# HowToSD/cremage

Hardware: AMD Instinct MI355X
Metric: images/sec SD1.5 512x512 20-step Euler ancestral (txt2img, CFG 7.5, incl. VAE decode) (higher is better)
Workload: dtype bf16; 1 GPU; SD1.5 txt2img 512x512, batch 4 per GPU, 20-step Euler ancestral, bf16 UNet (B=8 with CFG) + fp32-class (split-bf16 x3) VAE decode, synthetic name-keyed weights, synthetic conditioning; sampler=euler_a, sampler_steps=20, parallelism=batch-sharded x1 (weights broadcast 0.00 GB once, images all-gathered per step)

## Files before the change

### cremage_amd/_lib.py

```python
import ctypes as C
import os

_HERE = os.path.dirname(os.path.abspath(__file__))
HALF_F16 = os.environ.get("CRG_HALF", "bf16").lower() in ("f16", "fp16", "float16", "half")
LIB_PATH = os.path.abspath(os.environ["CRG_LIB"]) if os.environ.get("CRG_LIB") else os.path.join(_HERE, "libcrg_hip_f16.so" if HALF_F16 else "libcrg_hip.so")

BF16, F32, F16 = 0, 1, 2
PREC_BF16, PREC_BF16X3, PREC_F16MX = 0, 1, 2
EPI_NONE, EPI_SILU, EPI_GEGLU = 0, 1, 2
BIAS_NONE, BIAS_COL, BIAS_ROW = 0, 1, 2
PACK_LINEAR, PACK_CONV, PACK_GEGLU, PACK_CONV_UP2, PACK_CONVT_UP2 = 0, 1, 2, 3, 4
K_SLOTS = 17
SLOT_NAMES = ["gemm_w1", "gemm_w4", "gemm_w5", "gemm_x3", "conv_w1", "conv_w4", "conv_w5", "conv_x3", "splitk_reduce", "attention",
              "gn_stats", "gn_apply", "layernorm", "elementwise", "conv_small", "softmax", "lngemm"]
SLOT_FAMILY = ["gemm", "gemm", "gemm", "gemm", "conv", "conv", "conv", "conv", "splitk_reduce", "attention", "groupnorm", "groupnorm",
               "layernorm", "elementwise", "conv_small", "softmax", "gemm"]

c_void_p, c_int, c_int64, c_float, c_size_t = C.c_void_p, C.c_int, C.c_int64, C.c_float, C.c_size_t


class GemmArgs(C.Structure):
    _fields_ = [
        ("a", c_void_p), ("lda", c_int64), ("a_bstride", c_int64),
        ("w", c_void_p), ("ldw", c_int64), ("w_bstride", c_int64),
# ... 243 lines not shown
                                    c_int, c_float, c_int]),
    "crg_groupnorm_pre_split": (c_int, [c_void_p, c_void_p, c_void_p, c_void_p, c_void_p, c_void_p, c_void_p, c_void_p, c_int, c_int, c_int, c_int,
                                        c_float, c_int]),
    "crg_groupnorm_pre": (c_int, [c_void_p, c_void_p, c_void_p, c_void_p, c_int, c_void_p, c_void_p, c_void_p, c_void_p, c_void_p, c_int, c_int,
                                  c_int, c_int, c_float, c_int, c_int, c_int, c_int]),
    "crg_split_bf16": (c_int, [c_void_p, c_void_p, c_void_p, c_void_p, c_void_p, c_int64]),
    "crg_split_mx": (c_int, [c_void_p, c_void_p, c_void_p, c_void_p, c_void_p, c_int64, c_int, c_int, c_int]),
    "crg_groupnorm_mx": (c_int, [c_void_p, c_void_p, c_void_p, c_void_p, c_void_p, c_void_p, c_void_p, c_void_p, c_int, c_int, c_int, c_int, c_float,
                                 c_int, c_int, c_int]),
    "crg_pack_weight_mx": (c_int, [c_void_p, c_void_p, c_void_p, c_int, c_int, c_int, c_void_p, c_void_p, c_int, c_int]),
    "crg_layernorm": (c_int, [c_void_p, c_void_p, c_void_p, c_void_p, c_void_p, c_void_p, c_int64, c_int, c_float, c_int]),
    "crg_gemm": (c_int, [c_void_p, c_void_p, C.POINTER(GemmArgs)]),
    "crg_conv2d": (c_int, [c_void_p, c_void_p, C.POINTER(ConvArgs)]),
    "crg_last_route": (c_int, [c_void_p, C.POINTER(Route)]),
    "crg_ln_gemm": (c_int, [c_void_p, c_void_p, C.POINTER(LnGemmArgs)]),
    "crg_pack_weight": (c_int, [c_void_p, c_void_p, c_void_p, c_int, c_int, c_int, c_int, c_int, c_void_p, c_void_p]),
    "crg_pack_geglu_bias": (c_int, [c_void_p, c_void_p, c_void_p, c_int, c_void_p]),
    "crg_pack_ln_weight": (c_int, [c_void_p, c_void_p, c_void_p, c_int, c_void_p, c_void_p, c_void_p, c_int, c_int, c_int, c_void_p, c_void_p, c_void_p]),
    "crg_attention": (c_int, [c_void_p, c_void_p, c_void_p, c_int64, c_void_p, c_int64, c_void_p, c_int64, c_void_p, c_int64,
                              c_int, c_int, c_int, c_int, c_int, c_float, c_int]),
    "crg_attention_v": (c_int, [c_void_p, c_void_p, c_void_p, c_int64, c_void_p, c_int64, c_void_p, c_int64, c_void_p, c_int64,
                              c_int, c_int, c_int, c_int, c_int, c_float, c_int]),
    "crg_softmax_rows": (c_int, [c_void_p, c_void_p, c_void_p, c_void_p, c_int64, c_int, c_int64, c_float, c_int]),
    "crg_conv_small": (c_int, [c_void_p, c_void_p, c_void_p, c_void_p, c_void_p, c_void_p, c_int, c_int, c_int, c_int, c_int,
                               c_int, c_int, c_int]),
    "crg_timestep_embedding": (c_int, [c_void_p, c_void_p, c_void_p, c_void_p, c_int, c_int, c_int]),
    "crg_silu": (c_int, [c_void_p, c_void_p, c_void_p, c_void_p, c_int64, c_int]),
    "crg_nchw_to_nhwc": (c_int, [c_void_p, c_void_p, c_void_p, c_void_p, c_int, c_int, c_int, c_int, c_int]),
    "crg_nhwc_to_nchw": (c_int, [c_void_p, c_void_p, c_void_p, c_void_p, c_int, c_int, c_int, c_int, c_int]),
    "crg_nchw2_to_nhwc": (c_int, [c_void_p, c_void_p, c_void_p, c_void_p, c_void_p, c_int, c_int, c_int, c_int, c_int, c_int]),
# ... 131 lines not shown
```

### cremage_amd/csrc/crg_common.h

```cpp
#pragma once
#include <hip/hip_runtime.h>
#include <stdint.h>
#include <stdarg.h>
#include <stdio.h>
#include <string>
#include <vector>

#include "../../include/crg_hip.h"

#ifdef CRG_F16_BUILD
typedef _Float16 bf16;
#define CRG_HALF_KIND 1
#define CRG_MFMA_16x16x32(a, b, c) __builtin_amdgcn_mfma_f32_16x16x32_f16(a, b, c, 0, 0, 0)
#define CRG_MFMA_32x32x16(a, b, c) __builtin_amdgcn_mfma_f32_32x32x16_f16(a, b, c, 0, 0, 0)
#else
typedef __bf16 bf16;
#define CRG_HALF_KIND 0
#define CRG_MFMA_16x16x32(a, b, c) __builtin_amdgcn_mfma_f32_16x16x32_bf16(a, b, c, 0, 0, 0)
#define CRG_MFMA_32x32x16(a, b, c) __builtin_amdgcn_mfma_f32_32x32x16_bf16(a, b, c, 0, 0, 0)
#endif
typedef bf16 bf16x2 __attribute__((ext_vector_type(2)));
typedef bf16 bf16x4 __attribute__((ext_vector_type(4)));
typedef bf16 bf16x8 __attribute__((ext_vector_type(8)));
typedef float f32x2 __attribute__((ext_vector_type(2)));
// ... 38 lines not shown
  ~crg_prof_scope();
};

#define CRG_CHECK_LAUNCH(ctx, what)                                                    \
  do {                                                                                 \
    hipError_t e_ = hipGetLastError();                                                 \
    if (e_ != hipSuccess) return crg_fail(ctx, -5, "%s: launch failed: %s", what, hipGetErrorString(e_)); \
  } while (0)

#define CRG_REQUIRE(ctx, cond, ...)                         \
  do {                                                      \
    if (!(cond)) return crg_fail(ctx, -22, __VA_ARGS__);    \
  } while (0)

static inline size_t crg_dtype_size(int dt) { return dt == CRG_F32 ? 4 : 2; }

static inline int crg_set_dyn_lds(crg_ctx* ctx, const void* kern, size_t bytes, const char* what) {
  for (const void* k : ctx->lds_attr)
    if (k == kern) return 0;
  hipError_t e = hipFuncSetAttribute(kern, hipFuncAttributeMaxDynamicSharedMemorySize, (int)bytes);
  if (e != hipSuccess) return crg_fail(ctx, -5, "%s: cannot set %zu B dynamic LDS: %s", what, bytes, hipGetErrorString(e));
  ctx->lds_attr.push_back(kern);
  return 0;
}

__device__ __forceinline__ float crg_silu_f(float x) { return x * __builtin_amdgcn_rcpf(1.0f + __expf(-x)); }
__device__ __forceinline__ float crg_erf_f(float x) {
  const float ax = __builtin_fabsf(x);
  const float t = __builtin_amdgcn_rcpf(__builtin_fmaf(0.3275911f, ax, 1.0f));
  float q = __builtin_fmaf(1.061405429f, t, -1.453152027f);
// ... 72 lines not shown
```

### cremage_amd/csrc/lngemm.hip

```cpp
#include "gemm_shared.h"
#include <stdlib.h>

namespace crg_mm {

struct LnGemmP {
  const bf16* x; long ldx;
  const float* gamma; const float* beta; float eps;
  const bf16* w; long ldw;
  const float* bias;
  const bf16* res; long ldr; unsigned res_bytes;
  bf16* y; long ldy;
  int M, N, K, epi;
  unsigned x_bytes, w_bytes, y_bytes;
  bf16* vt; int vt_n0, vt_T; long vt_ld; unsigned vt_bytes;
};

#ifdef CRG_LN_ABL_NOSTORE
constexpr bool LN_DROP8 = true;
#else
constexpr bool LN_DROP8 = false;
#endif
static __device__ __forceinline__ void ln_wait(int n) {
  switch (n) {
    case 0: wait_vmcnt<0>(); break;
    case 1: wait_vmcnt<1>(); break;
    case 2: wait_vmcnt<2>(); break;
    case 3: wait_vmcnt<3>(); break;
    case 4: wait_vmcnt<4>(); break;
    case 5: wait_vmcnt<5>(); break;
// ... 40 lines not shown
    case 46: wait_vmcnt<46>(); break;
    case 47: wait_vmcnt<47>(); break;
    default: wait_vmcnt<0>(); break;
  }
}

template <int EXTRA>
static __device__ __forceinline__ void ln_wait_nw(int nW) {
  if (nW == 2) wait_vmcnt<2 + EXTRA>();
  else if (nW == 3) wait_vmcnt<3 + EXTRA>();
  else if (nW == 4) wait_vmcnt<4 + EXTRA>();
  else if (nW == 1) wait_vmcnt<1 + EXTRA>();
  else ln_wait(nW + EXTRA);
}

template <int WNT, int KT, bool GEGLU>
__global__ __launch_bounds__(512, 2) void lngemm_kernel(LnGemmP p) {
  constexpr bool PAIR = !GEGLU;
  constexpr int WMT = 2, NW = 8, BMR = 128, WST = 4;
  constexpr int BN = 32 * WNT;
  constexpr int WS_BYTES = BN * 128;
  constexpr int WRG = BN / 8;
  constexpr int WL = (WRG + NW - 1) / NW;
  constexpr int A_KT = BMR * 128;
  constexpr int AP = KT * 16 / NW;
  static_assert((KT * 16) % NW == 0, "A pieces must divide over the waves");
  constexpr int OOB = (int)0x80000000;
  extern __shared__ __attribute__((aligned(16))) char smem[];
  char* const Ares = smem;
  char* const wring = smem + KT * A_KT;

  const int t = threadIdx.x;
  const int lane = t & 63;
  const int wave = __builtin_amdgcn_readfirstlane(t >> 6);
  const int wm = wave >> 1, wn = wave & 1;
  const int m0 = blockIdx.x * BMR;
  const int rsub = lane >> 3;
  const int clog = (lane & 7) ^ rsub;
  const int frow = lane & 15, fq = lane >> 4;
  const int nW = (WRG - wave + NW - 1) / NW;
  const int tiles_n = (p.N + BN - 1) / BN;
  const int U = tiles_n * KT;
  constexpr int NST = GEGLU ? WMT * (WNT / 2) : WMT * (WNT / 2 + (WNT & 1));
  constexpr int NSTT = WMT * (8 * (WNT / 2) + 4 * (WNT & 1));

#pragma unroll
  for (int i = 0; i < AP; ++i) {
    const int pa = wave + NW * i;
    const int kt = pa >> 4, rg = pa & 15;
    const int row = m0 + rg * 8 + rsub;
    const int vo = row < p.M ? (int)((long)row * p.ldx * 2) + clog * 16 : OOB;
    buf_dma16(p.x, p.x_bytes, Ares + kt * A_KT + rg * 1024, vo, kt * 128);
  }
  int wvo[WL];
#pragma unroll
  for (int q = 0; q < WL; ++q) {
    const int pos = (wave + NW * q) * 8 + rsub;
    const int nl = PAIR ? unpair_col<WNT>(pos) : pos;
    wvo[q] = (wave + NW * q) < WRG ? (int)((long)nl * p.ldw * 2) + clog * 16 : OOB;
  }
  auto stage_w = [&](int u) {
    const int nt = u / KT, kt = u - nt * KT;
    char* ws = wring + (u & 3) * WS_BYTES;
    const int soff = (int)((long)nt * BN * p.ldw * 2) + kt * 128;
#pragma unroll
    for (int q = 0; q < WL; ++q)
      if ((wave + NW * q) < WRG) buf_dma16(p.w, p.w_bytes, ws + (wave + NW * q) * 1024, wvo[q], soff);
  };
  stage_w(0);
  stage_w(1);
  stage_w(2);

  if (p.gamma) {
    const int c = lane & 7, r8 = lane >> 3;
    f32x4 g0[KT], g1[KT], b0[KT], b1[KT];
#pragma unroll
    for (int kt = 0; kt < KT; ++kt) {
      const int k = kt * 64 + c * 8;
      g0[kt] = *reinterpret_cast<const f32x4*>(p.gamma + k);
      g1[kt] = *reinterpret_cast<const f32x4*>(p.gamma + k + 4);
      b0[kt] = *reinterpret_cast<const f32x4*>(p.beta + k);
      b1[kt] = *reinterpret_cast<const f32x4*>(p.beta + k + 4);
    }
    ln_wait(nW * 3);
    asm volatile("" ::: "memory");
    __builtin_amdgcn_s_barrier();
    asm volatile("" ::: "memory");
    const float inv_k = 1.0f / (float)(KT * 64);
// ... 30 lines not shown
#pragma unroll
        for (int e = 0; e < 8; ++e) {
          const float ga = e < 4 ? g0[kt][e] : g1[kt][e - 4], be = e < 4 ? b0[kt][e] : b1[kt][e - 4];
          o[e] = (bf16)(((float)v[kt][e] - mean) * rstd * ga + be);
        }
        *reinterpret_cast<bf16x8*>(Ares + kt * A_KT + lds_off(row, c)) = o;
      }
    }
  }

  f32x4 acc[WNT][WMT];
#pragma unroll
  for (int i = 0; i < WNT; ++i)
#pragma unroll
    for (int j = 0; j < WMT; ++j) acc[i][j] = f32x4{0.f, 0.f, 0.f, 0.f};
  const int wb0 = (wn * (16 * WNT) + frow) * 128 + ((fq ^ (frow & 7)) << 4);
  int aoff[WMT];
#pragma unroll
  for (int j = 0; j < WMT; ++j) aoff[j] = lds_off(wm * 32 + j * 16 + frow, fq);

  bf16x8 xa[KT][2][WMT];
  bf16x8 wf0[WNT], wf1[WNT];
  auto read_frags = [&](bf16x8 (&wf)[WNT], int slot, int ks) {
    const char* wbase = wring + slot * WS_BYTES + (wb0 ^ (ks << 6));
#pragma unroll
    for (int i = 0; i < WNT; ++i) wf[i] = *reinterpret_cast<const bf16x8*>(wbase + i * 2048);
  };
  auto mma = [&](const bf16x8 (&xf)[WMT], const bf16x8 (&wf)[WNT]) {
#pragma unroll
    for (int i = 0; i < WNT; ++i)
#pragma unroll
      for (int j = 0; j < WMT; ++j) acc[i][j] = CRG_MFMA_16x16x32(wf[i], xf[j], acc[i][j]);
  };
  {
    ln_wait(nW * 2);
    asm volatile("" ::: "memory");
    __builtin_amdgcn_s_barrier();
    asm volatile("" ::: "memory");
#pragma unroll
    for (int kt = 0; kt < KT; ++kt)
#pragma unroll
      for (int ks = 0; ks < 2; ++ks)
#pragma unroll
        for (int j = 0; j < WMT; ++j) xa[kt][ks][j] = *reinterpret_cast<const bf16x8*>(Ares + kt * A_KT + (aoff[j] ^ (ks << 6)));
    read_frags(wf0, 0, 0);
  }
  for (int nt = 0; nt < tiles_n; ++nt) {
// ... 14 lines not shown
      asm volatile("" ::: "memory");
      __builtin_amdgcn_s_barrier();
      asm volatile("" ::: "memory");
      read_frags(wf1, u & 3, 1);
      __builtin_amdgcn_sched_barrier(0);
#ifndef CRG_LN_ABL_NOMMA
      mma(xa[kt][0], wf0);
#endif
      __builtin_amdgcn_sched_barrier(0);
#ifndef CRG_LN_ABL_NODMA
      stage_w(u + 3);
#endif
      read_frags(wf0, (u + 1) & 3, 0);
      __builtin_amdgcn_sched_barrier(0);
#ifndef CRG_LN_ABL_NOMMA
      mma(xa[kt][1], wf1);
#else
      asm volatile("" ::"v"(wf1[0]), "v"(wf0[0]));
#endif
    }
    {
      constexpr int OOBS = (int)0x80000000;
      const int nb = n0 + wn * (16 * WNT);
      if constexpr (GEGLU) {
#pragma unroll
        for (int u2 = 0; u2 < WNT / 2; ++u2) {
          const int pn = nb + u2 * 32 + fq * 4;
          const int jn = nb / 2 + u2 * 16 + fq * 4;
          const bool nok = pn + 20 <= p.N;
          f32x4 bv = {0.f, 0.f, 0.f, 0.f}, bg = bv;
          if (p.bias) {
            const int pc = nok ? pn : 0;
            bv = *reinterpret_cast<const f32x4*>(p.bias + pc);
            bg = *reinterpret_cast<const f32x4*>(p.bias + pc + 16);
          }
#pragma unroll
          for (int j = 0; j < WMT; ++j) {
            const int m = m0 + wm * 32 + j * 16 + frow;
            const f32x4 v = acc[2 * u2][j] + bv, g = acc[2 * u2 + 1][j] + bg;
            bf16x4 o;
#pragma unroll
            for (int e = 0; e < 4; ++e) o[e] = (bf16)(v[e] * crg_gelu_erf_f(g[e]));
            buf_store8<LN_DROP8>(p.y, p.y_bytes, (nok && m < p.M) ? (int)(((long)m * p.ldy + jn) * 2) : OOBS, o);
          }
        }
      } else if (p.vt && n0 >= p.vt_n0) {
        const int Cv = p.N - p.vt_n0;
#pragma unroll
        for (int j = 0; j < WMT; ++j) {
          const int m = m0 + wm * 32 + j * 16 + frow;
          const int bs = m / p.vt_T, tk = m - bs * p.vt_T;
          const long row0 = (long)bs * Cv - p.vt_n0;
#pragma unroll
          for (int u2 = 0; u2 < WNT / 2; ++u2) {
            const int n = nb + 32 * u2 + 8 * fq;
#pragma unroll
            for (int e = 0; e < 8; ++e) {
              const float v = e < 4 ? acc[2 * u2][j][e] : acc[2 * u2 + 1][j][e - 4];
              const float bsv = p.bias ? p.bias[n + e < p.N ? n + e : 0] : 0.f;
// ... 359 lines not shown
    CRG_CHECK_LAUNCH(ctx, "ln_gemm");
    return 0;
  }
  if (geglu) { kern = lngemm_kernel<4, 5, true>; bn = 128; }
  else if (wide) { kern = lngemm_kernel<5, 5, false>; bn = 160; }
  else { kern = lngemm_kernel<4, 5, false>; bn = 128; }
  const size_t lds = (size_t)5 * 128 * 128 + (size_t)4 * bn * 128;
  if (int rc = crg_set_dyn_lds(ctx, reinterpret_cast<const void*>(kern), 160 * 1024, "ln_gemm")) return rc;
  const double flops = 2.0 * a->M * (double)a->N * a->K;
  const double bytes = (double)a->M * a->K * 2 + (double)a->N * a->K * 2 + (double)a->M * n_out * 2;
  crg_prof_scope ps(ctx, st, CRG_K_LNGEMM, flops, bytes);
  hipLaunchKernelGGL(kern, dim3((a->M + 127) / 128), dim3(512), lds, st, p);
  CRG_CHECK_LAUNCH(ctx, "ln_gemm");
  return 0;
}
```

### cremage_amd/csrc/norms.hip

```cpp
#include "crg_common.h"
#include <cstdlib>

namespace {

constexpr int GN_MAX_GROUPS = 32;
constexpr int GN_TILE_MAX_C = 1280;

template <typename T>
__global__ __launch_bounds__(512) void gn_stats_kernel(const T* __restrict__ x, const T* __restrict__ x2, int C1, int C, int HW,
                                                       int groups, int rows_per_chunk, float* __restrict__ part,
                                                       float* __restrict__ kbuf) {
  __shared__ float shiftv[GN_MAX_GROUPS];
  const int n = blockIdx.y, chunk = blockIdx.x;
  const int tpr = C >> 3;
  const int rpi = blockDim.x / tpr;
  const int t = threadIdx.x;
  const int col = t % tpr, rl = t / tpr;
  const int gs = C / groups;
  const int C2 = C - C1;
  if (t < groups) {
    const int c = t * gs;
    shiftv[t] = (c < C1) ? (float)x[(long)n * HW * C1 + c] : (float)x2[(long)n * HW * C2 + (c - C1)];
    if (chunk == 0) kbuf[n * groups + t] = shiftv[t];
  }
// ... 625 lines not shown
    while ((long)chunks * crg_heur_samples(ctx, N) < 512 && chunks * 8 <= HW && chunks < 256) chunks *= 2;
    const int rpc = (HW + chunks - 1) / chunks;
    chunks = (HW + rpc - 1) / rpc;
    crg_prof_scope ps(ctx, st, CRG_K_GN_APPLY, 5.0 * elems, elems * 4.0);
    if (fold_in_apply)
      hipLaunchKernelGGL(gn_apply_kernel<bf16>, dim3(chunks, N), dim3(threads), 0, st, (const bf16*)x, (const bf16*)x2, C1, C, HW, groups, rpc, -rows1,
                         stats1, stats2, gamma, beta, eps, fuse_silu, (bf16*)y, (bf16*)nullptr, (bf16*)nullptr, (unsigned char*)nullptr, 0.f, 0.f, rows2);
    else
      hipLaunchKernelGGL(gn_apply_kernel<bf16>, dim3(chunks, N), dim3(threads), 0, st, (const bf16*)x, (const bf16*)x2, C1, C, HW, groups, rpc, -1,
                         mr, (const float*)nullptr, gamma, beta, eps, fuse_silu, (bf16*)y, (bf16*)nullptr, (bf16*)nullptr);
  }
  CRG_CHECK_LAUNCH(ctx, "groupnorm_pre");
  return 0;
}

extern "C" int crg_groupnorm_pre_split(crg_ctx* ctx, void* stream, const void* x, const float* stats, const float* gamma, const float* beta,
                                       void* y_hi, void* y_lo, int N, int HW, int C, int groups, float eps, int fuse_silu) {
  if (!ctx) return -22;
  CRG_REQUIRE(ctx, N > 0 && HW > 0 && C > 0 && x && stats, "groupnorm_pre_split: empty input");
  CRG_REQUIRE(ctx, y_hi && y_lo && (((uintptr_t)y_hi | (uintptr_t)y_lo | (uintptr_t)x | (uintptr_t)stats) & 15) == 0, "groupnorm_pre_split: pointers must be 16-byte aligned");
  CRG_REQUIRE(ctx, groups > 0 && groups <= GN_MAX_GROUPS && C % groups == 0, "groupnorm_pre_split: groups=%d C=%d unsupported", groups, C);
  CRG_REQUIRE(ctx, C % 8 == 0 && (C >> 3) <= 512, "groupnorm_pre_split: C=%d must be a multiple of 8 and <= 4096", C);
  CRG_REQUIRE(ctx, HW % 32 == 0, "groupnorm_pre_split: HW=%d must be a multiple of the 32-row statistics blocks", HW);
  CRG_REQUIRE(ctx, C / groups <= 128, "groupnorm_pre_split: group size %d unsupported (<= 128)", C / groups);
  const long rbs = (long)N * (HW >> 5);
  float* mr = (float*)crg_scratch(ctx, (size_t)N * groups * 2 * sizeof(float));
  if (!mr) return crg_fail(ctx, -12, "groupnorm_pre_split: out of scratch");
  hipStream_t st = (hipStream_t)stream;
  const double elems = (double)N * HW * C;
  {
// ... 100 lines not shown
```

### cremage_amd/knobs.py

```python
import os

GN_STATS = os.environ.get("CRG_GN_STATS", "1") != "0"
VAE_GN_STATS = os.environ.get("CRG_VAE_GN_STATS", "1") != "0"
GN_TILE = os.environ.get("CRG_GN_TILE", "1") != "0"
LN_EPI = os.environ.get("CRG_LN_EPI", "1") != "0"
LN_EPI_320 = int(os.environ.get("CRG_LN_EPI_320", "1"))
LN_EPI_MASK = int(os.environ.get("CRG_LN_EPI_MASK", "3"))
VAE_MX = os.environ.get("CRG_VAE_MX", "0") != "0"
FF_MX8 = os.environ.get("CRG_FF_MX8", "0") != "0"
ATTN_X3_FLASH = os.environ.get("CRG_ATTN_X3", "0") != "0"
SCORE_BUDGET_BYTES = 256 << 20
CFG_SHARE = os.environ.get("CRG_CFG_SHARE", "1") != "0"
TIME_ROWS = os.environ.get("CRG_TIME_ROWS", "1") != "0"
UP_SUBPIX = os.environ.get("CRG_UP_SUBPIX", "1") != "0"
SELF_QKV = os.environ.get("CRG_SELF_QKV", "1") != "0"
STEP_TABLES = os.environ.get("CRG_SAMPLER_TABLES", "1") != "0"
```

### cremage_amd/ldm_hip/transformer.py

```python
from __future__ import annotations

from typing import List, Optional

import torch
import torch.nn as nn

from .. import knobs, ops
from .nn import Conv2d, Linear, Normalize, zero_module


def exists(v):
    return v is not None


def default(v, d):
    return v if exists(v) else d


def zero_init_module(module):
    for p in module.parameters():
        p.data.zero_()
    return module


# ... 265 lines not shown
        self.transformer_blocks = nn.ModuleList([
            BasicTransformerBlock(inner_dim, n_heads, d_head, dropout=dropout, context_dim=context_dim[d],
                                  disable_self_attn=disable_self_attn, checkpoint=use_checkpoint, lora_ranks=self.lora_ranks,
                                  lora_weights=self.lora_weights, ipa_scale=ipa_scale, ipa_num_tokens=ipa_num_tokens)
            for d in range(depth)])
        self.proj_out = zero_module(Conv2d(inner_dim, in_channels, kernel_size=1, stride=1, padding=0))
        _lora_lists(self, "proj_out", inner_dim, in_channels, self.lora_ranks, conv=True)

    def cfg_dup_ok(self) -> bool:
        return len(self.transformer_blocks) > 0 and self.transformer_blocks[0].cfg_dup_ok()

    def forward(self, x, context=None, cfg_dup: bool = False):
        x = ops.to_channels_last(x)
        b, c, h, w = x.shape
        x_in = ops.tokens_of(x)
        xn = self.norm(x)
        t = ops.linear(ops.tokens_of(xn), _eff(self, self.proj_in.weight, "proj_in"), self.proj_in.bias,
                       row_stats=ops.ln_epi_wanted(self.proj_in.weight.shape[0]))
        nb = len(self.transformer_blocks)
        for i, block in enumerate(self.transformer_blocks):
            block._crg_next_is_block = i + 1 < nb
            if cfg_dup and i == 0:
                t = block(t, context=context, cfg_dup=True)
                x_in = ops.dup_batch(x_in)
                continue
            t = block(t, context=context)
        y = ops.linear(t, _eff(self, self.proj_out.weight, "proj_out"), self.proj_out.bias, residual=x_in, gn_hw=h * w)
        return ops.image_of_stats(y, h, w)
```

### cremage_amd/ops/__init__.py

```python
from .. import knobs
from ._base import (HALF, TensorKeyedCache, _h, _st, clear_weight_cache, empty_image, f32_vec, image_of, image_of_stats,
                    nchw_to_nhwc, nhwc_to_nchw, profile, to_channels_last, tokens_of)
from .attn import attention, attention_rows_v, attention_x3_ok
from .conv import affine_cast, conv1x1, conv2d, mx_conv_ok, split_bf16, upsample_subpixel_ok
from .film import avg_pool2, flow_up2_add, leaky_split, scale_into, warp_flow
from .frames import MAX_FRAMES, add_frames, attention_frames, blend_frames, conv_frames, conv_frames_thin, conv_frames_x3, frames_weight, lincomb_frames
from .gemm import _gemm, last_route, linear, linear_transposed, linear_transposed_ok, ln_linear, ln_linear_auto, ln_linear_ok, rows_per_sample
from .imaging import (BLEND_GRAY, RESAMPLE_BITS, bilinear_tables, blur_blend_u8, lanczos_tables, paste_warped_u8, poisson_clone, poisson_tables, resample_u8,
                      upscale_noise, upscaled_size, warp_affine_u8)
from .mx8 import dequant_mx8_host, ff_mx8_ok, linear_mx8, linear_mx8_host, packed_weight_mx8, quant_mx8, quant_mx8_host
from .norms import group_norm, layer_norm, softmax_rows_
from .packing import MX_X_LOG2, packed_geglu_bias, packed_ln_weight, packed_weight, packed_weight_mx, split_mx
from .side_channels import (GN_STATS_MIN_HW, _gn_rows_of, _gn_stats_of, attach_time_rows, dup_batch, ln_epi_ok, ln_epi_wanted,
                            mark_cfg_dup, row_stats_parts, time_rows_of)
from .unblur import conv_transpose2d, group_norm_add_act
from .steps import KSTEP_KINDS, STEP_KINDS, axpby_, cfg_ddim_step_, cfg_dpmpp2m_step_, cfg_euler_step_, cfg_kstep_, cfg_sampler_step_, silu, timestep_embedding

__all__ = [
    "BLEND_GRAY", "GN_STATS_MIN_HW", "HALF", "KSTEP_KINDS", "MAX_FRAMES", "MX_X_LOG2", "RESAMPLE_BITS", "STEP_KINDS", "TensorKeyedCache", "add_frames",
    "affine_cast", "attach_time_rows", "attention", "attention_frames", "attention_rows_v", "attention_x3_ok", "avg_pool2", "axpby_", "bilinear_tables",
    "blend_frames", "blur_blend_u8", "cfg_ddim_step_", "cfg_dpmpp2m_step_", "cfg_euler_step_", "cfg_kstep_", "cfg_sampler_step_", "clear_weight_cache",
    "conv1x1", "conv2d", "conv_transpose2d", "conv_frames", "conv_frames_thin", "conv_frames_x3", "dequant_mx8_host", "dup_batch", "empty_image", "f32_vec", "ff_mx8_ok",
    "flow_up2_add", "frames_weight", "group_norm", "group_norm_add_act", "image_of", "image_of_stats", "lanczos_tables", "last_route", "layer_norm", "leaky_split",
    "lincomb_frames", "linear", "linear_mx8", "linear_mx8_host", "linear_transposed", "linear_transposed_ok", "ln_epi_ok", "ln_epi_wanted", "ln_linear",
    "ln_linear_auto", "ln_linear_ok", "mark_cfg_dup", "mx_conv_ok", "nchw_to_nhwc", "nhwc_to_nchw", "packed_geglu_bias", "packed_ln_weight",
    "packed_weight", "packed_weight_mx", "packed_weight_mx8", "paste_warped_u8", "poisson_clone", "poisson_tables", "profile", "quant_mx8", "quant_mx8_host",
    "resample_u8", "row_stats_parts", "rows_per_sample", "scale_into", "silu", "softmax_rows_", "split_bf16", "split_mx", "time_rows_of",
    "timestep_embedding", "to_channels_last", "tokens_of", "upsample_subpixel_ok", "upscale_noise", "upscaled_size", "warp_affine_u8", "warp_flow",
]
```

### cremage_amd/ops/gemm.py

```python
import ctypes as C
import math
from typing import Optional

import torch

from .. import _lib as L, knobs
from ._base import _DT, HALF, _act_dt, _call, _h, _need_cuda, _p, _prec, _st, f32_vec
from .norms import layer_norm
from .packing import packed_geglu_bias, packed_ln_weight, packed_weight
from .side_channels import _gn_stats_buffer, _ln_stats_of, ln_epi_ok, row_stats_parts


def _gemm(h, **kw):
    a = L.GemmArgs()
    for k, v in kw.items():
        setattr(a, k, v)
    L.check(L.load().crg_gemm(h, _st(), C.byref(a)), h, "crg_gemm")


def rows_per_sample(x: torch.Tensor, gn_hw: Optional[int] = None) -> int:
    if gn_hw:
        return int(gn_hw)
    return 1 if x.dim() <= 2 else int(math.prod(x.shape[1:-1]))


# ... 125 lines not shown
        ld = (tokens + 7) // 8 * 8
        vt = torch.empty((x.shape[0], N - transposed_from, ld), dtype=x.dtype, device=x.device)
        if ld != tokens:
            vt[:, :, tokens:].zero_()
    if residual is not None:
        residual = residual.contiguous()
        if residual.shape != y.shape or residual.dtype != y.dtype:
            raise L.CrgError("ln_linear: residual must match the output in shape and dtype")
    a = L.LnGemmArgs(x=x.data_ptr(), ldx=K, gamma=_p(f32_vec(ln_weight)).value, beta=_p(f32_vec(ln_bias)).value, eps=float(eps),
                     w=hi.data_ptr(), ldw=K, bias=_p(b).value, y=y.data_ptr(), ldy=n_out, M=M, N=N, K=K, epilogue=L.EPI_GEGLU if geglu else L.EPI_NONE,
                     vt=_p(vt).value, vt_n0=transposed_from or 0, vt_tokens=tokens, vt_ld=ld, residual=_p(residual).value, ldr=n_out)
    _call("crg_ln_gemm", x, C.byref(a))
    return (y, vt) if transposed_from is not None else y


def linear_transposed(x: torch.Tensor, weight: torch.Tensor, bias: Optional[torch.Tensor] = None) -> torch.Tensor:
    _need_cuda(x, weight, bias)
    x = x.contiguous()
    B, T, K = x.shape
    N = weight.shape[0]
    split = x.dtype == torch.float32
    hi, lo = packed_weight(weight, L.PACK_LINEAR, split)
    ld = (T + 7) // 8 * 8
    y = torch.empty((B, N, ld), dtype=x.dtype, device=x.device)
    if ld != T:
        y[:, :, T:].zero_()
    b = f32_vec(bias)
    h = _h(x)
    xh, xl = x, None
    if split:
# ... 8 lines not shown
```

### include/crg_hip.h

```cpp
#ifndef CRG_HIP_H
#define CRG_HIP_H

#include <stddef.h>
#include <stdint.h>

#ifdef __cplusplus
extern "C" {
#endif

#define CRG_VERSION 104

typedef struct crg_ctx crg_ctx;

enum crg_dtype { CRG_BF16 = 0, CRG_F32 = 1, CRG_F16 = 2 };

enum crg_prec { CRG_PREC_BF16 = 0, CRG_PREC_BF16X3 = 1,
                CRG_PREC_F16MX = 2 };

enum crg_epilogue {
  CRG_EPI_NONE = 0,
  CRG_EPI_SILU = 1,
  CRG_EPI_GEGLU = 2
};

// ... 49 lines not shown
int crg_layernorm(crg_ctx* ctx, void* stream, const void* x, const float* gamma, const float* beta, void* y,
                  int64_t rows, int dim, float eps, int dtype);

typedef struct {
  const void* x; int64_t ldx;
  const float* gamma; const float* beta; float eps;
  const void* w; int64_t ldw;
  const float* bias;
  void* y; int64_t ldy;
  int M, N, K;
  int epilogue;
  void* vt; int vt_n0; int vt_tokens; int64_t vt_ld;
  const void* residual; int64_t ldr;
} crg_lngemm_args;
int crg_ln_gemm(crg_ctx* ctx, void* stream, const crg_lngemm_args* args);

typedef struct {
  const void* a; int64_t lda; int64_t a_bstride;
  const void* w; int64_t ldw; int64_t w_bstride;
  const void* w_lo;
  const float* bias; int bias_mode;
  const void* residual; int64_t ldr; int64_t r_bstride;
  void* y; int64_t ldy; int64_t y_bstride;
  int M, N, K, batch;
  int epilogue;
  int a_dtype, y_dtype, prec;
  int a_is_weight;
  const void* a_lo;
  float* gn_stats;
  void* vt; int vt_n0; int vt_tokens; int64_t vt_ld;
// ... 316 lines not shown
```

Baseline: 17.98 images/s.

## Fuse GroupNorm into the proj_in GEMM for 320-channel spatial transformers

Adds a GroupNorm variant of the row-resident LN-GEMM kernel. It folds the precomputed per-tile GroupNorm partial statistics into per-group mean/rstd inside the block, normalizes the A tile in LDS, then runs the proj_in GEMM with a row-stats epilogue. Transformer proj_in at C=320 uses it when the stats side channel is available. This removes the separate GroupNorm apply kernel and its activation round trip through memory, at the cost of extra in-kernel reduction work and a narrow supported shape.

```diff
diff --git a/cremage_amd/_lib.py b/cremage_amd/_lib.py
--- a/cremage_amd/_lib.py
+++ b/cremage_amd/_lib.py
@@ -281,6 +281,8 @@
     "crg_conv2d": (c_int, [c_void_p, c_void_p, C.POINTER(ConvArgs)]),
     "crg_last_route": (c_int, [c_void_p, C.POINTER(Route)]),
     "crg_ln_gemm": (c_int, [c_void_p, c_void_p, C.POINTER(LnGemmArgs)]),
+    "crg_gn_gemm": (c_int, [c_void_p, c_void_p, c_void_p, c_void_p, c_int, c_void_p, c_void_p, c_int, c_float, c_void_p, c_void_p, c_void_p, c_void_p, c_int,
+                            c_int, c_int, c_int, c_int]),
     "crg_pack_weight": (c_int, [c_void_p, c_void_p, c_void_p, c_int, c_int, c_int, c_int, c_int, c_void_p, c_void_p]),
     "crg_pack_geglu_bias": (c_int, [c_void_p, c_void_p, c_void_p, c_int, c_void_p]),
     "crg_pack_ln_weight": (c_int, [c_void_p, c_void_p, c_void_p, c_int, c_void_p, c_void_p, c_void_p, c_int, c_int, c_int, c_void_p, c_void_p, c_void_p]),
diff --git a/cremage_amd/csrc/crg_common.h b/cremage_amd/csrc/crg_common.h
--- a/cremage_amd/csrc/crg_common.h
+++ b/cremage_amd/csrc/crg_common.h
@@ -76,6 +76,8 @@
   } while (0)
 
 static inline size_t crg_dtype_size(int dt) { return dt == CRG_F32 ? 4 : 2; }
+
+int crg_gn_stats_for_consumer(crg_ctx* ctx, hipStream_t st, const float* stats, int N, int HW, int C, int groups, float eps, int rows, const float** mr);
 
 static inline int crg_set_dyn_lds(crg_ctx* ctx, const void* kern, size_t bytes, const char* what) {
   for (const void* k : ctx->lds_attr)
diff --git a/cremage_amd/csrc/lngemm.hip b/cremage_amd/csrc/lngemm.hip
--- a/cremage_amd/csrc/lngemm.hip
+++ b/cremage_amd/csrc/lngemm.hip
@@ -13,6 +13,8 @@
   int M, N, K, epi;
   unsigned x_bytes, w_bytes, y_bytes;
   bf16* vt; int vt_n0, vt_T; long vt_ld; unsigned vt_bytes;
+  const float* gn_stat; long gn_plane; int gn_tiles, gn_hw, gn_groups;
+  float* rstat; int rstat_parts; unsigned rstat_bytes;
 };
 
 #ifdef CRG_LN_ABL_NOSTORE
@@ -83,8 +85,10 @@
   else ln_wait(nW + EXTRA);
 }
 
-template <int WNT, int KT, bool GEGLU>
+template <int WNT, int KT, bool GEGLU, bool GN = false, bool KG2 = false>
 __global__ __launch_bounds__(512, 2) void lngemm_kernel(LnGemmP p) {
+  static_assert(!GN || (!GEGLU && WNT == 5), "the GroupNorm form is the plain 160-column tile (its scratch lies in ring slot 3)");
+  static_assert(!KG2 || GN, "two k-groups: the GroupNorm form only");
   constexpr bool PAIR = !GEGLU;
   constexpr int WMT = 2, NW = 8, BMR = 128, WST = 4;
   constexpr int BN = 32 * WNT;
@@ -110,7 +114,7 @@
   const int nW = (WRG - wave + NW - 1) / NW;
   const int tiles_n = (p.N + BN - 1) / BN;
   const int U = tiles_n * KT;
-  constexpr int NST = GEGLU ? WMT * (WNT / 2) : WMT * (WNT / 2 + (WNT & 1));
+  constexpr int NST = (GEGLU ? WMT * (WNT / 2) : WMT * (WNT / 2 + (WNT & 1))) + (GN ? WMT : 0);
   constexpr int NSTT = WMT * (8 * (WNT / 2) + 4 * (WNT & 1));
 
 #pragma unroll
@@ -140,7 +144,96 @@
   stage_w(1);
   stage_w(2);
 
-  if (p.gamma) {
+  if constexpr (GN) {
+    constexpr int C = KT * 64, NQ = C / 4, TS = 256 / NQ;
+    static_assert((2 * TS * C + 64 + 2 * C) * 4 <= WS_BYTES, "the GroupNorm scratch must fit one ring slot");
+    float* const csum = reinterpret_cast<float*>(wring + 3 * WS_BYTES);
+    float* const meanv = csum + 2 * TS * C;
+    float* const rstdv = meanv + 32;
+    float* const scv = rstdv + 32;
+    float* const sfv = scv + C;
+    const int smp = m0 / p.gn_hw;
+    const int groups = p.gn_groups, gs = C / groups;
+    float ga = 0.f, be = 0.f;
+    if (t < C) {
+      ga = p.gamma[t];
+      be = p.beta[t];
+    }
+    if (p.gn_tiles > 0) {
+      if (t < NQ * TS) {
+        const int ts = t / NQ, c = (t - ts * NQ) * 4;
+        const float* q = p.gn_stat + c + (long)smp * p.gn_tiles * C;
+        f32x4 a = {0.f, 0.f, 0.f, 0.f}, b = a;
+#pragma unroll 4
+        for (int i = ts; i < p.gn_tiles; i += TS) {
+          a += *reinterpret_cast<const f32x4*>(q + (long)i * C);
+          b += *reinterpret_cast<const f32x4*>(q + (long)i * C + p.gn_plane);
+        }
+        *reinterpret_cast<f32x4*>(csum + ts * C + c) = a;
+        *reinterpret_cast<f32x4*>(csum + TS * C + ts * C + c) = b;
+      }
+    } else if (t < groups) {
+      meanv[t] = p.gn_stat[((long)smp * groups + t) * 2];
+      rstdv[t] = p.gn_stat[((long)smp * groups + t) * 2 + 1];
+    }
+    auto lds_barrier = [&]() {
+      wait_lgkmcnt0();
+      asm volatile("" ::: "memory");
+      __builtin_amdgcn_s_barrier();
+      asm volatile("" ::: "memory");
+    };
+    ln_wait(nW * 3);
+    lds_barrier();
+    if (p.gn_tiles > 0) {
+      if (t < groups) {
+        double da = 0.0, db = 0.0;
+        for (int ts = 0; ts < TS; ++ts)
+          for (int cl = 0; cl < gs; ++cl) {
+            da += (double)csum[ts * C + t * gs + cl];
+            db += (double)csum[TS * C + ts * C + t * gs + cl];
+          }
+        const double cnt = (double)p.gn_hw * gs;
+        const double md = da / cnt;
+        double var = db / cnt - md * md;
+        if (var < 0.0) var = 0.0;
+        meanv[t] = (float)md;
+        rstdv[t] = (float)(1.0 / sqrt(var + (double)p.eps));
+      }
+      lds_barrier();
+    }
+    if (t < C) {
+      const int g = t / gs;
+      scv[t] = rstdv[g] * ga;
+      sfv[t] = be - meanv[g] * rstdv[g] * ga;
+    }
+    lds_barrier();
+    const int c = lane & 7, r8 = lane >> 3;
+    f32x4 s0[KT], s1[KT], f0[KT], f1[KT];
+#pragma unroll
+    for (int kt = 0; kt < KT; ++kt) {
+      const int k = kt * 64 + c * 8;
+      s0[kt] = *reinterpret_cast<const f32x4*>(scv + k);
+      s1[kt] = *reinterpret_cast<const f32x4*>(scv + k + 4);
+      f0[kt] = *reinterpret_cast<const f32x4*>(sfv + k);
+      f1[kt] = *reinterpret_cast<const f32x4*>(sfv + k + 4);
+    }
+#pragma unroll
+    for (int it = 0; it < 2; ++it) {
+      const int row = wave * 16 + it * 8 + r8;
+#pragma unroll
+      for (int kt = 0; kt < KT; ++kt) {
+        const bf16x8 v = *reinterpret_cast<const bf16x8*>(Ares + kt * A_KT + lds_off(row, c));
+        bf16x8 o;
+#pragma unroll
+        for (int e = 0; e < 8; ++e) {
+          const float sc = e < 4 ? s0[kt][e] : s1[kt][e - 4], sf = e < 4 ? f0[kt][e] : f1[kt][e - 4];
+          o[e] = (bf16)((float)v[e] * sc + sf);
+        }
+        *reinterpret_cast<bf16x8*>(Ares + kt * A_KT + lds_off(row, c)) = o;
+      }
+    }
+    wait_lgkmcnt0();
+  } else if (p.gamma) {
     const int c = lane & 7, r8 = lane >> 3;
     f32x4 g0[KT], g1[KT], b0[KT], b1[KT];
 #pragma unroll
@@ -201,6 +294,13 @@
   for (int i = 0; i < WNT; ++i)
 #pragma unroll
     for (int j = 0; j < WMT; ++j) acc[i][j] = f32x4{0.f, 0.f, 0.f, 0.f};
+  f32x4 acc1[KG2 ? WNT : 1][KG2 ? WMT : 1];
+  if constexpr (KG2) {
+#pragma unroll
+    for (int i = 0; i < WNT; ++i)
+#pragma unroll
+      for (int j = 0; j < WMT; ++j) acc1[i][j] = f32x4{0.f, 0.f, 0.f, 0.f};
+  }
   const int wb0 = (wn * (16 * WNT) + frow) * 128 + ((fq ^ (frow & 7)) << 4);
   int aoff[WMT];
 #pragma unroll
@@ -218,6 +318,14 @@
     for (int i = 0; i < WNT; ++i)
 #pragma unroll
       for (int j = 0; j < WMT; ++j) acc[i][j] = CRG_MFMA_16x16x32(wf[i], xf[j], acc[i][j]);
+  };
+  auto mma1 = [&](const bf16x8 (&xf)[WMT], const bf16x8 (&wf)[WNT]) {
+    if constexpr (KG2) {
+#pragma unroll
+      for (int i = 0; i < WNT; ++i)
+#pragma unroll
+        for (int j = 0; j < WMT; ++j) acc1[i][j] = CRG_MFMA_16x16x32(wf[i], xf[j], acc1[i][j]);
+    }
   };
   {
     ln_wait(nW * 2);
@@ -262,7 +370,8 @@
       read_frags(wf0, (u + 1) & 3, 0);
       __builtin_amdgcn_sched_barrier(0);
 #ifndef CRG_LN_ABL_NOMMA
-      mma(xa[kt][1], wf1);
+      if constexpr (KG2) mma1(xa[kt][1], wf1);
+      else mma(xa[kt][1], wf1);
 #else
       asm volatile("" ::"v"(wf1[0]), "v"(wf0[0]));
 #endif
@@ -291,6 +400,72 @@
             for (int e = 0; e < 4; ++e) o[e] = (bf16)(v[e] * crg_gelu_erf_f(g[e]));
             buf_store8<LN_DROP8>(p.y, p.y_bytes, (nok && m < p.M) ? (int)(((long)m * p.ldy + jn) * 2) : OOBS, o);
           }
+        }
+      } else if constexpr (GN) {
+        const int part = (nt * 2 + wn) * 2;
+        if constexpr (KG2) {
+#pragma unroll
+          for (int i = 0; i < WNT; ++i)
+#pragma unroll
+            for (int j = 0; j < WMT; ++j) {
+              acc[i][j] += acc1[i][j];
+              acc1[i][j] = f32x4{0.f, 0.f, 0.f, 0.f};
+            }
+        }
+#pragma unroll
+        for (int j = 0; j < WMT; ++j) {
+          const int m = m0 + wm * 32 + j * 16 + frow;
+          float q1 = 0.f, q2 = 0.f;
+#pragma unroll
+          for (int u2 = 0; u2 < WNT / 2; ++u2) {
+            const int n = nb + 32 * u2 + 8 * fq;
+            const bool nok = n + 8 <= p.N;
+            f32x4 ba = {0.f, 0.f, 0.f, 0.f}, bb = ba;
+            if (p.bias) {
+              const int pc = nok ? n : 0;
+              ba = *reinterpret_cast<const f32x4*>(p.bias + pc);
+              bb = *reinterpret_cast<const f32x4*>(p.bias + pc + 4);
+            }
+            const f32x4 a4 = acc[2 * u2][j] + ba, b4 = acc[2 * u2 + 1][j] + bb;
+            bf16x8 o;
+#pragma unroll
+            for (int e = 0; e < 4; ++e) {
+              o[e] = (bf16)a4[e];
+              o[4 + e] = (bf16)b4[e];
+            }
+            buf_store16(p.y, p.y_bytes, (nok && m < p.M) ? (int)(((long)m * p.ldy + n) * 2) : OOBS, o);
+#pragma unroll
+            for (int e = 0; e < 8; ++e) {
+              const float f = nok ? (float)o[e] : 0.f;
+              q1 += f;
+              q2 = __builtin_fmaf(f, f, q2);
+            }
+          }
+          if constexpr (WNT & 1) {
+            const int n = nb + 16 * (WNT - 1) + 4 * fq;
+            const bool nok = n + 4 <= p.N;
+            f32x4 ba = {0.f, 0.f, 0.f, 0.f};
+            if (p.bias) ba = *reinterpret_cast<const f32x4*>(p.bias + (nok ? n : 0));
+            const f32x4 a4 = acc[WNT - 1][j] + ba;
+            bf16x4 o;
+#pragma unroll
+            for (int e = 0; e < 4; ++e) o[e] = (bf16)a4[e];
+            buf_store8<LN_DROP8>(p.y, p.y_bytes, (nok && m < p.M) ? (int)(((long)m * p.ldy + n) * 2) : OOBS, o);
+#pragma unroll
+            for (int e = 0; e < 4; ++e) {
+              const float f = nok ? (float)o[e] : 0.f;
+              q1 += f;
+              q2 = __builtin_fmaf(f, f, q2);
+            }
+          }
+          q1 += __shfl_xor(q1, 16);
+          q2 += __shfl_xor(q2, 16);
+          q1 += __shfl_xor(q1, 32);
+          q2 += __shfl_xor(q2, 32);
+          const f32x2 qq = {q1, q2};
+          bf16x4 raw;
+          __builtin_memcpy(&raw, &qq, 8);
+          buf_store8<false>(p.rstat, p.rstat_bytes, (fq == 0 && m < p.M) ? (int)(((long)m * p.rstat_parts * 2 + part) * 4) : OOBS, raw);
         }
       } else if (p.vt && n0 >= p.vt_n0) {
         const int Cv = p.N - p.vt_n0;
@@ -680,3 +855,49 @@
   CRG_CHECK_LAUNCH(ctx, "ln_gemm");
   return 0;
 }
+
+extern "C" int crg_gn_gemm(crg_ctx* ctx, void* stream, const void* x, const float* gn_stats, int gn_stats_rows, const float* gamma, const float* beta,
+                           int groups, float eps, const void* w, const float* bias, void* y, float* row_stats, int row_stats_parts, int N, int HW,
+                           int C, int n_out) {
+  if (!ctx) return -22;
+  CRG_REQUIRE(ctx, N > 0 && HW > 0 && n_out > 0 && x && w && y && gamma && beta && gn_stats, "gn_gemm: empty problem N=%d HW=%d n_out=%d", N, HW, n_out);
+  CRG_REQUIRE(ctx, C == 320, "gn_gemm: the row-resident kernel is built for C = 320 (got %d): use crg_groupnorm_pre + crg_gemm", C);
+  CRG_REQUIRE(ctx, HW % 128 == 0, "gn_gemm: HW=%d must be a multiple of the 128-row block (a block lies inside one sample)", HW);
+  CRG_REQUIRE(ctx, n_out % 160 == 0, "gn_gemm: n_out=%d must be a multiple of the 160-column tile", n_out);
+  CRG_REQUIRE(ctx, (((uintptr_t)x | (uintptr_t)w | (uintptr_t)y | (uintptr_t)gamma | (uintptr_t)beta | (uintptr_t)bias | (uintptr_t)gn_stats | (uintptr_t)row_stats) & 15) == 0,
+              "gn_gemm: pointers must be 16-byte aligned");
+  const double M = (double)N * HW;
+  CRG_REQUIRE(ctx, M * C * 2.0 < 2147483648.0 && M * n_out * 2.0 < 2147483648.0, "gn_gemm: operands must be < 2 GiB");
+  if (row_stats) {
+    CRG_REQUIRE(ctx, row_stats_parts == 2 * (n_out / 160), "gn_gemm: row_stats_parts = 2 * n_out / 160 = %d (got %d)", 2 * (n_out / 160), row_stats_parts);
+    CRG_REQUIRE(ctx, M * row_stats_parts * 8.0 < 2147483648.0, "gn_gemm: row statistics must be < 2 GiB");
+  }
+  hipStream_t st = (hipStream_t)stream;
+  const float* mr = nullptr;
+  if (int rc = crg_gn_stats_for_consumer(ctx, st, gn_stats, N, HW, C, groups, eps, gn_stats_rows, &mr)) return rc;
+  LnGemmP p{};
+  p.x = (const bf16*)x; p.ldx = C; p.gamma = gamma; p.beta = beta; p.eps = eps;
+  p.w = (const bf16*)w; p.ldw = C; p.bias = bias; p.y = (bf16*)y; p.ldy = n_out;
+  p.M = N * HW; p.N = n_out; p.K = C; p.epi = CRG_EPI_NONE;
+  p.x_bytes = (unsigned)(M * C * 2.0); p.w_bytes = (unsigned)((double)n_out * C * 2.0); p.y_bytes = (unsigned)(M * n_out * 2.0);
+  p.gn_hw = HW; p.gn_groups = groups;
+  if (mr) { p.gn_stat = mr; p.gn_tiles = 0; p.gn_plane = 0; }
+  else { p.gn_stat = gn_stats; p.gn_tiles = HW / gn_stats_rows; p.gn_plane = (long)N * (HW >> 5) * C; }
+  if (row_stats) { p.rstat = row_stats; p.rstat_parts = row_stats_parts; p.rstat_bytes = (unsigned)(M * row_stats_parts * 8.0); }
+  crg_gemm_args ga{};
+  ga.a = x; ga.lda = C; ga.w = w; ga.ldw = C; ga.bias = bias; ga.bias_mode = bias ? CRG_BIAS_COL : CRG_BIAS_NONE; ga.y = y; ga.ldy = n_out;
+  ga.M = p.M; ga.N = n_out; ga.K = C; ga.batch = 1; ga.epilogue = CRG_EPI_NONE; ga.a_dtype = CRG_BF16; ga.y_dtype = CRG_BF16; ga.prec = CRG_PREC_BF16;
+  ga.row_stats = row_stats; ga.row_stats_parts = row_stats ? row_stats_parts : 0; ga.rows_per_sample = HW;
+  const crg_plan::Plan pl = crg_plan::plan_gemm(ga, crg_plan::Env{ctx->invariant, ctx->n_cu, dev_knobs()});
+  if (pl.rc) return crg_fail(ctx, pl.rc, "gn_gemm: %s", pl.msg);
+  const bool kg2 = pl.main.family == crg_plan::F_GLDS && pl.main.cfg == 3;
+  void (*kern)(LnGemmP) = kg2 ? lngemm_kernel<5, 5, false, true, true> : lngemm_kernel<5, 5, false, true, false>;
+  const size_t lds = (size_t)5 * 128 * 128 + (size_t)4 * 160 * 128;
+  if (int rc = crg_set_dyn_lds(ctx, reinterpret_cast<const void*>(kern), 160 * 1024, "gn_gemm")) return rc;
+  const double flops = 2.0 * M * (double)n_out * C;
+  const double bytes = M * C * 2 + (double)n_out * C * 2 + M * n_out * 2;
+  crg_prof_scope ps(ctx, st, CRG_K_LNGEMM, flops, bytes);
+  hipLaunchKernelGGL(kern, dim3((p.M + 127) / 128), dim3(512), lds, st, p);
+  CRG_CHECK_LAUNCH(ctx, "gn_gemm");
+  return 0;
+}
diff --git a/cremage_amd/csrc/norms.hip b/cremage_amd/csrc/norms.hip
--- a/cremage_amd/csrc/norms.hip
+++ b/cremage_amd/csrc/norms.hip
@@ -663,6 +663,23 @@
   return 0;
 }
 
+int crg_gn_stats_for_consumer(crg_ctx* ctx, hipStream_t st, const float* stats, int N, int HW, int C, int groups, float eps, int rows, const float** mr_out) {
+  CRG_REQUIRE(ctx, groups > 0 && groups <= GN_MAX_GROUPS && C % groups == 0 && C / groups <= 128, "gn_gemm: groups=%d C=%d unsupported", groups, C);
+  CRG_REQUIRE(ctx, stats && rows > 0 && rows % 32 == 0 && HW % rows == 0, "gn_gemm: rows per partial (%d) must be a multiple of 32 that divides HW=%d", rows, HW);
+  const long fold_floats = (long)(HW / rows) * C;
+  const bool fold_in_apply = rows >= 64 && C <= GN_TILE_MAX_C && fold_floats <= 10240 && ((uintptr_t)stats & 15) == 0;
+  *mr_out = nullptr;
+  if (fold_in_apply) return 0;
+  const long rbs = (long)N * (HW >> 5);
+  float* mr = (float*)crg_scratch(ctx, (size_t)N * groups * 2 * sizeof(float));
+  if (!mr) return crg_fail(ctx, -12, "gn_gemm: out of scratch");
+  crg_prof_scope ps(ctx, st, CRG_K_GN_STATS, 2.0 * rbs * C, 8.0 * rbs * C);
+  hipLaunchKernelGGL(gn_finalize_kernel, dim3(groups, N), dim3(256), 0, st, stats, (const float*)nullptr, C, C, HW, groups, rbs * C, 0L, eps, mr, rows, 32);
+  CRG_CHECK_LAUNCH(ctx, "gn_gemm(finalize)");
+  *mr_out = mr;
+  return 0;
+}
+
 extern "C" int crg_groupnorm_pre_split(crg_ctx* ctx, void* stream, const void* x, const float* stats, const float* gamma, const float* beta,
                                        void* y_hi, void* y_lo, int N, int HW, int C, int groups, float eps, int fuse_silu) {
   if (!ctx) return -22;
diff --git a/cremage_amd/knobs.py b/cremage_amd/knobs.py
--- a/cremage_amd/knobs.py
+++ b/cremage_amd/knobs.py
@@ -15,3 +15,7 @@
 UP_SUBPIX = os.environ.get("CRG_UP_SUBPIX", "1") != "0"
 SELF_QKV = os.environ.get("CRG_SELF_QKV", "1") != "0"
 STEP_TABLES = os.environ.get("CRG_SAMPLER_TABLES", "1") != "0"
+
+
+class chain:
+    GN_PROJ_IN = os.environ.get("CRG_GN_PROJ_IN", "1") != "0"
diff --git a/cremage_amd/ldm_hip/transformer.py b/cremage_amd/ldm_hip/transformer.py
--- a/cremage_amd/ldm_hip/transformer.py
+++ b/cremage_amd/ldm_hip/transformer.py
@@ -303,9 +303,12 @@
         x = ops.to_channels_last(x)
         b, c, h, w = x.shape
         x_in = ops.tokens_of(x)
-        xn = self.norm(x)
-        t = ops.linear(ops.tokens_of(xn), _eff(self, self.proj_in.weight, "proj_in"), self.proj_in.bias,
-                       row_stats=ops.ln_epi_wanted(self.proj_in.weight.shape[0]))
+        w_in = _eff(self, self.proj_in.weight, "proj_in")
+        st = ops.ln_epi_wanted(self.proj_in.weight.shape[0])
+        if ops.gn_linear_ok(x, self.norm.weight, self.norm.num_groups, w_in):
+            t = ops.gn_linear(x, self.norm.weight, self.norm.bias, self.norm.num_groups, self.norm.eps, w_in, self.proj_in.bias, row_stats=st)
+        else:
+            t = ops.linear(ops.tokens_of(self.norm(x)), w_in, self.proj_in.bias, row_stats=st)
         nb = len(self.transformer_blocks)
         for i, block in enumerate(self.transformer_blocks):
             block._crg_next_is_block = i + 1 < nb
diff --git a/cremage_amd/ops/__init__.py b/cremage_amd/ops/__init__.py
--- a/cremage_amd/ops/__init__.py
+++ b/cremage_amd/ops/__init__.py
@@ -5,7 +5,7 @@
 from .conv import affine_cast, conv1x1, conv2d, mx_conv_ok, split_bf16, upsample_subpixel_ok
 from .film import avg_pool2, flow_up2_add, leaky_split, scale_into, warp_flow
 from .frames import MAX_FRAMES, add_frames, attention_frames, blend_frames, conv_frames, conv_frames_thin, conv_frames_x3, frames_weight, lincomb_frames
-from .gemm import _gemm, last_route, linear, linear_transposed, linear_transposed_ok, ln_linear, ln_linear_auto, ln_linear_ok, rows_per_sample
+from .gemm import _gemm, gn_linear, gn_linear_ok, last_route, linear, linear_transposed, linear_transposed_ok, ln_linear, ln_linear_auto, ln_linear_ok, rows_per_sample
 from .imaging import (BLEND_GRAY, RESAMPLE_BITS, bilinear_tables, blur_blend_u8, lanczos_tables, paste_warped_u8, poisson_clone, poisson_tables, resample_u8,
                       upscale_noise, upscaled_size, warp_affine_u8)
 from .mx8 import dequant_mx8_host, ff_mx8_ok, linear_mx8, linear_mx8_host, packed_weight_mx8, quant_mx8, quant_mx8_host
@@ -21,7 +21,7 @@
     "affine_cast", "attach_time_rows", "attention", "attention_frames", "attention_rows_v", "attention_x3_ok", "avg_pool2", "axpby_", "bilinear_tables",
     "blend_frames", "blur_blend_u8", "cfg_ddim_step_", "cfg_dpmpp2m_step_", "cfg_euler_step_", "cfg_kstep_", "cfg_sampler_step_", "clear_weight_cache",
     "conv1x1", "conv2d", "conv_transpose2d", "conv_frames", "conv_frames_thin", "conv_frames_x3", "dequant_mx8_host", "dup_batch", "empty_image", "f32_vec", "ff_mx8_ok",
-    "flow_up2_add", "frames_weight", "group_norm", "group_norm_add_act", "image_of", "image_of_stats", "lanczos_tables", "last_route", "layer_norm", "leaky_split",
+    "flow_up2_add", "frames_weight", "gn_linear", "gn_linear_ok", "group_norm", "group_norm_add_act", "image_of", "image_of_stats", "lanczos_tables", "last_route", "layer_norm", "leaky_split",
     "lincomb_frames", "linear", "linear_mx8", "linear_mx8_host", "linear_transposed", "linear_transposed_ok", "ln_epi_ok", "ln_epi_wanted", "ln_linear",
     "ln_linear_auto", "ln_linear_ok", "mark_cfg_dup", "mx_conv_ok", "nchw_to_nhwc", "nhwc_to_nchw", "packed_geglu_bias", "packed_ln_weight",
     "packed_weight", "packed_weight_mx", "packed_weight_mx8", "paste_warped_u8", "poisson_clone", "poisson_tables", "profile", "quant_mx8", "quant_mx8_host",
diff --git a/cremage_amd/ops/gemm.py b/cremage_amd/ops/gemm.py
--- a/cremage_amd/ops/gemm.py
+++ b/cremage_amd/ops/gemm.py
@@ -8,7 +8,7 @@
 from ._base import _DT, HALF, _act_dt, _call, _h, _need_cuda, _p, _prec, _st, f32_vec
 from .norms import layer_norm
 from .packing import packed_geglu_bias, packed_ln_weight, packed_weight
-from .side_channels import _gn_stats_buffer, _ln_stats_of, ln_epi_ok, row_stats_parts
+from .side_channels import _gn_rows_of, _gn_stats_buffer, _gn_stats_of, _ln_stats_of, ln_epi_ok, row_stats_parts
 
 
 def _gemm(h, **kw):
@@ -164,6 +164,37 @@
     return (y, vt) if transposed_from is not None else y
 
 
+def gn_linear_ok(x: torch.Tensor, gn_weight: torch.Tensor, groups: int, weight: torch.Tensor) -> bool:
+    if not (knobs.chain.GN_PROJ_IN and x.is_cuda and x.dim() == 4 and x.dtype == HALF and x.shape[1] == 320 and weight[0].numel() == 320):
+        return False
+    n, c, hh, ww = x.shape
+    hw = hh * ww
+    if hw % 128 or weight.shape[0] % 160 or gn_weight.numel() != c or not (0 < groups <= 32) or c % groups:
+        return False
+    if not x.permute(0, 2, 3, 1).is_contiguous() or _gn_stats_of(x, hw) is None or hw % _gn_rows_of(x):
+        return False
+    return L.invariant() > 0 or n * hw * max(c, weight.shape[0]) * 2 < (1 << 31)
+
+
+def gn_linear(x: torch.Tensor, gn_weight, gn_bias, groups: int, eps: float, weight: torch.Tensor, bias: Optional[torch.Tensor] = None,
+              row_stats: bool = False) -> torch.Tensor:
+    _need_cuda(x, gn_weight, gn_bias, weight, bias)
+    if not gn_linear_ok(x, gn_weight, groups, weight):
+        raise L.CrgError("gn_linear: outside the fused kernel's domain (test gn_linear_ok, else group_norm + linear)")
+    n, c, hh, ww = x.shape
+    hw, n_out = hh * ww, weight.shape[0]
+    hi, _ = packed_weight(weight, L.PACK_LINEAR, False)
+    y = torch.empty((n, hw, n_out), dtype=x.dtype, device=x.device)
+    rs = None
+    if row_stats and knobs.LN_EPI and row_stats_parts(n_out) <= 16:
+        rs = torch.empty((n * hw, row_stats_parts(n_out), 2), dtype=torch.float32, device=x.device)
+    _call("crg_gn_gemm", x, _p(x), _p(_gn_stats_of(x, hw)), _gn_rows_of(x), _p(f32_vec(gn_weight)), _p(f32_vec(gn_bias)), int(groups), float(eps),
+          _p(hi), _p(f32_vec(bias)), _p(y), _p(rs), rs.shape[1] if rs is not None else 0, n, hw, c, n_out)
+    if rs is not None:
+        y._crg_ln = (rs, y._version)
+    return y
+
+
 def linear_transposed(x: torch.Tensor, weight: torch.Tensor, bias: Optional[torch.Tensor] = None) -> torch.Tensor:
     _need_cuda(x, weight, bias)
     x = x.contiguous()
diff --git a/include/crg_hip.h b/include/crg_hip.h
--- a/include/crg_hip.h
+++ b/include/crg_hip.h
@@ -87,6 +87,10 @@
   const void* residual; int64_t ldr;
 } crg_lngemm_args;
 int crg_ln_gemm(crg_ctx* ctx, void* stream, const crg_lngemm_args* args);
+
+int crg_gn_gemm(crg_ctx* ctx, void* stream, const void* x, const float* gn_stats, int gn_stats_rows, const float* gamma, const float* beta,
+                int groups, float eps, const void* w, const float* bias, void* y, float* row_stats, int row_stats_parts, int N, int HW,
+                int C, int n_out);
 
 typedef struct {
   const void* a; int64_t lda; int64_t a_bstride;
```

New measurement: 18.04 images/s (median of 6 runs). Within noise of the previous version (+0.4%).
